# bayespy/bayespy

Hardware: AMD Instinct MI355X
Metric: VB iterations/sec, PCA N=10000000 D=128 K=32 (higher is better)
Workload: dtype f64

## Files before the change

### bayespy_amd/csrc/vmp_common.h

```cpp
#pragma once

#include <hip/hip_runtime.h>
#include <stdint.h>
#include <stdio.h>
#include <string.h>
#include <math.h>

#include "../../include/vmp_hip.h"

#define VMP_EV_RING 64

constexpr int VMP_NME = 16;

struct vmp_xpass_desc {
    const double *Y;
    int64_t ldy, N;
    int D, K;
    double *X;
    int64_t ldx;
    int lay;
    const double *A;
    int buf;
};

struct vmp_ctx {
    int device;
    hipStream_t stream;
    int num_cu;
    int timing;
    hipEvent_t ev[3 * VMP_EV_RING];
    int64_t ev_n;
    hipStream_t xs;
    hipEvent_t ev_xfork, ev_xdone;
    int x_pending;
    hipEvent_t ev_xbuf[2];
    int x_buf_pending[2];
    int64_t x_count;
    int xs_cus;
    int x_hold, x_held;
    vmp_xpass_desc x_desc;
    int64_t x_launched, x_superseded;
    double *sweep_ctl;
    int64_t sweeps_enqueued;
    unsigned int *sweep_tickets;
    int64_t sweep_mid_launches;
    unsigned long long *sweep_stamps;
    int sweep_stamp_rows;
    hipStream_t ms[3];
    hipEvent_t me[VMP_NME];
    int gram_pending;
    int gram_D, gram_K;
    double *gram_state;
    double *gram_P;
    void *comm;
    int comm_rank, comm_world;
    void *queue;
    char err[512];
};

enum { VMP_SWEEP_NSTAMP = VMP_PCA_SWEEP_NSTAMP };

enum { VMP_SWEEP_STOP = 0, VMP_SWEEP_L = 1, VMP_SWEEP_EXECUTED = 2, VMP_SWEEP_SKIPPED = 3,
       VMP_SWEEP_CTL_LEN = 8 };

struct vmp_sweep_tail {
    const double *P;
    int nb;
    double *ctl;
    double *slot;
    int first;
    int compare;
    double l0, tol;
    int norder;
    int order[8];
};

int32_t vmp_pca_sweep_covered(int32_t D, int32_t K);
int32_t vmp_pca_launch_sweep_head(vmp_ctx *ctx, int32_t D, int32_t K, int64_t n_total, double x_prec,
                                  double a0t, double b0t, double a0a, double b0a, double *state,
                                  const double *stop);
int32_t vmp_pca_launch_sweep_tail(vmp_ctx *ctx, int32_t D, int32_t K, int64_t n_total, double x_prec,
                                  double a0t, double b0t, double a0a, double b0a, double *state,
                                  const vmp_sweep_tail &t);

int32_t vmp_pca_launch_sweep_mid(vmp_ctx *ctx, int32_t D, int32_t K, int64_t n_total, double x_prec,
                                 double a0t, double b0t, double a0a, double b0a, double *state,
                                 double *P, const vmp_sweep_tail &t, unsigned int *ticket, int32_t wide,
                                 unsigned long long *stamps);
int32_t vmp_pca_launch_sweep_head_wide(vmp_ctx *ctx, int32_t D, int32_t K, int64_t n_total,
                                       double x_prec, double a0t, double b0t, double a0a, double b0a,
                                       double *state);
int32_t vmp_pca_launch_gram_fast(vmp_ctx *ctx, int32_t D, int32_t K, double *state, double *P,
                                 int32_t wide);

int32_t vmp_pca_ensure_gram(vmp_ctx *ctx);
int32_t vmp_pca_launch_held(vmp_ctx *ctx);

int32_t vmp_queue_flush(vmp_ctx *ctx);
int32_t vmp_queue_commit(vmp_ctx *ctx);
int32_t destroy_small_queue(vmp_ctx *ctx);
extern const char *vmp_flush_cause;
#define VMP_FLUSH_SMALL(ctx)                                   \
    do {                                                       \
        if ((ctx) && (ctx)->queue) {                           \
            vmp_flush_cause = __func__;                        \
            const int32_t rc__ = vmp_queue_flush(ctx);         \
            if (rc__ != VMP_OK) return rc__;                   \
        }                                                      \
    } while (0)

static inline hipEvent_t *vmp_next_events(vmp_ctx *ctx)
// ... 258 lines not shown
```

### bayespy_amd/csrc/vmp_ctx.hip

```cpp
#include "vmp_common.h"

#include <new>

static char g_err[512] = "no context";

namespace {
struct tune_entry { char key[32]; int value; };
tune_entry g_tune[128];
int g_ntune = 0;
bool g_tune_env = false;
}

extern "C" char **environ;

static void tune_from_env()
{
    g_tune_env = true;
    for (char **e = environ; e && *e; ++e) {
        if (strncmp(*e, "VMP_TUNE_", 9) != 0) continue;
        const char *eq = strchr(*e, '=');
        if (!eq) continue;
        const size_t len = (size_t)(eq - (*e + 9));
        if (len == 0 || len >= sizeof(g_tune[0].key) || g_ntune >= (int)(sizeof(g_tune) / sizeof(g_tune[0])))
            continue;
// ... 52 lines not shown
    vmp_ctx *ctx = new (std::nothrow) vmp_ctx();
    if (!ctx) return VMP_ERR_HIP;
    ctx->device = device;
    ctx->stream = (hipStream_t)stream;
    ctx->timing = 0;
    ctx->err[0] = 0;
    for (int i = 0; i < 3 * VMP_EV_RING; ++i) ctx->ev[i] = nullptr;
    ctx->ev_n = 0;
    ctx->xs = nullptr;
    ctx->ev_xfork = ctx->ev_xdone = nullptr;
    ctx->x_pending = 0;
    ctx->x_buf_pending[0] = ctx->x_buf_pending[1] = 0;
    ctx->x_count = 0;
    ctx->ev_xbuf[0] = ctx->ev_xbuf[1] = nullptr;
    ctx->xs_cus = 0;
    ctx->x_hold = ctx->x_held = 0;
    ctx->x_launched = ctx->x_superseded = 0;
    ctx->sweep_ctl = nullptr;
    ctx->sweeps_enqueued = 0;
    ctx->sweep_tickets = nullptr;
    ctx->sweep_mid_launches = 0;
    ctx->sweep_stamps = nullptr;
    ctx->sweep_stamp_rows = 0;
    for (int i = 0; i < 3; ++i) ctx->ms[i] = nullptr;
    for (int i = 0; i < VMP_NME; ++i) ctx->me[i] = nullptr;
    ctx->comm = nullptr;
    ctx->queue = nullptr;
    ctx->comm_rank = 0;
    ctx->comm_world = 1;
    VMP_HIP_CHECK(ctx, hipSetDevice(device));
    int cu = 0;
    VMP_HIP_CHECK(ctx, hipDeviceGetAttribute(&cu, hipDeviceAttributeMultiprocessorCount, device));
    ctx->num_cu = cu > 0 ? cu : 256;
    *out = ctx;
    return VMP_OK;
}

int32_t vmp_ctx_destroy(vmp_ctx *ctx)
{
    if (!ctx) return VMP_OK;
    (void)destroy_small_queue(ctx);
    (void)vmp_comm_destroy(ctx);
    (void)vmp_pca_launch_held(ctx);
    for (int i = 0; i < 3 * VMP_EV_RING; ++i)
        if (ctx->ev[i]) (void)hipEventDestroy(ctx->ev[i]);
    if (ctx->xs) {
        (void)hipStreamSynchronize(ctx->xs);
        (void)hipStreamDestroy(ctx->xs);
    }
    for (int i = 0; i < 3; ++i)
        if (ctx->ms[i]) {
            (void)hipStreamSynchronize(ctx->ms[i]);
            (void)hipStreamDestroy(ctx->ms[i]);
        }
    for (int i = 0; i < VMP_NME; ++i)
        if (ctx->me[i]) (void)hipEventDestroy(ctx->me[i]);
    if (ctx->sweep_ctl) (void)hipFree(ctx->sweep_ctl);
    if (ctx->sweep_tickets) (void)hipFree(ctx->sweep_tickets);
    if (ctx->sweep_stamps) (void)hipFree(ctx->sweep_stamps);
    if (ctx->ev_xfork) (void)hipEventDestroy(ctx->ev_xfork);
    if (ctx->ev_xdone) (void)hipEventDestroy(ctx->ev_xdone);
    for (int i = 0; i < 2; ++i)
        if (ctx->ev_xbuf[i]) (void)hipEventDestroy(ctx->ev_xbuf[i]);
    delete ctx;
    return VMP_OK;
}

int32_t vmp_ctx_set_stream(vmp_ctx *ctx, void *stream)
{
    if (!ctx) return VMP_ERR_INVALID;
    if ((hipStream_t)stream != ctx->stream) VMP_FLUSH_SMALL(ctx);
    ctx->stream = (hipStream_t)stream;
    return VMP_OK;
}

int32_t vmp_ctx_sync(vmp_ctx *ctx)
{
    if (!ctx) return VMP_ERR_INVALID;
    VMP_FLUSH_SMALL(ctx);
    {
        const int32_t rcg = vmp_pca_ensure_gram(ctx);
        if (rcg != VMP_OK) return rcg;
// ... 261 lines not shown
```

### bayespy_amd/csrc/vmp_pca.hip

```cpp
#include "vmp_common.h"
#include "vmp_stop_rule.h"

namespace {

constexpr int TN = 32;
constexpr int SZ = TN + 2;
constexpr int NT = 256;
constexpr int MAX_KP = 64;
constexpr int MAX_DP = 256;

inline int pow2_blocks(int x, int unit)
{
    int b = (x + unit - 1) / unit;
    int p = 1;
    while (p < b) p <<= 1;
    return p;
}

inline void fill_layout(int D, int K, vmp_pca_layout *L)
{
    const int64_t DP = 32 * pow2_blocks(D, 32);
    const int64_t KP = 16 * pow2_blocks(K, 16);
    int64_t o = 0;
    L->DP = DP;
// ... 1129 lines not shown
    if (rc != VMP_OK) return rc;
    if (!ctx->sweep_ctl) {
        VMP_HIP_CHECK(ctx, hipMalloc(&ctx->sweep_ctl, VMP_SWEEP_CTL_LEN * sizeof(double)));
        VMP_HIP_CHECK(ctx, hipMemsetAsync(ctx->sweep_ctl, 0, VMP_SWEEP_CTL_LEN * sizeof(double),
                                          ctx->stream));
    }
    vmp_pca_layout L;
    fill_layout(D, K, &L);
    double *P = reinterpret_cast<double *>(workspace);
    vmp_sweep_tail t;
    t.P = P;
    t.nb = (int)(L.DP / GR);
    t.ctl = ctx->sweep_ctl;
    t.compare = compare ? 1 : 0;
    t.l0 = l0;
    t.tol = tol;
    t.norder = norder;
    for (int i = 0; i < 8; ++i) t.order[i] = i < norder ? order[i] : -1;
    const bool ticket = n > 1 && ((uintptr_t)state % 16) == 0 &&
                        vmp_tune_get("pca_sweep_ticket", env_int("VMP_PCA_SWEEP_TICKET", 1, 0, 1));
    int wide = vmp_tune_get("pca_sweep_wide", env_int("VMP_PCA_SWEEP_WIDE", 1, 0, 1)) ? 1 : 0;
    if (wide && vmp_tune_get("pca_sweep_local_pxx", env_int("VMP_PCA_SWEEP_LOCAL_PXX", 1, 0, 1)))
        wide = 2;
    const bool stamps = ticket && vmp_tune_get("pca_sweep_stamps", 0);
    if (stamps) {
        const size_t bytes = (size_t)VMP_PCA_MAX_SWEEPS * VMP_SWEEP_NSTAMP * sizeof(unsigned long long);
        if (!ctx->sweep_stamps) VMP_HIP_CHECK(ctx, hipMalloc(&ctx->sweep_stamps, bytes));
        VMP_HIP_CHECK(ctx, hipMemsetAsync(ctx->sweep_stamps, 0,
                                          (size_t)(n - 1) * VMP_SWEEP_NSTAMP * sizeof(unsigned long long),
                                          ctx->stream));
        ctx->sweep_stamp_rows = n - 1;
    }
    if (ticket) {
        if (!ctx->sweep_tickets) {
            VMP_HIP_CHECK(ctx, hipMalloc(&ctx->sweep_tickets,
                                         VMP_PCA_MAX_SWEEPS * sizeof(unsigned int)));
            VMP_HIP_CHECK(ctx, hipMemsetAsync(ctx->sweep_tickets, 0,
                                              VMP_PCA_MAX_SWEEPS * sizeof(unsigned int), ctx->stream));
        }
    }
    bool head_wide = ticket && wide;
    if (head_wide && ctx->x_pending) {
        head_wide = hipEventQuery(ctx->ev_xdone) == hipSuccess;
        (void)hipGetLastError();
    }
    for (int i = 0; i < n; ++i) {
        const double *stop = i == 0 ? nullptr : ctx->sweep_ctl;
        const bool last = i + 1 == n;
        if (i == 0 && head_wide) {
            rc = vmp_pca_launch_sweep_head_wide(ctx, D, K, n_total, x_prec, a0_tau, b0_tau, a0_alpha,
                                                b0_alpha, state);
            if (rc != VMP_OK) return rc;
        } else if (!ticket || i == 0) {
            rc = vmp_pca_launch_sweep_head(ctx, D, K, n_total, x_prec, a0_tau, b0_tau, a0_alpha,
                                           b0_alpha, state, stop);
            if (rc != VMP_OK) return rc;
        }
        if (last) {
            rc = issue_xpass(ctx, Y, ldy, N, D, K, X, ldx, state, workspace, lay);
            if (rc != VMP_OK) return rc;
        } else {
            ctx->x_superseded += 1;
        }
        t.slot = ring + (int64_t)i * VMP_PCA_SWEEP_SLOT;
        t.first = i == 0;
        if (ticket && !last) {
            rc = vmp_pca_launch_sweep_mid(ctx, D, K, n_total, x_prec, a0_tau, b0_tau, a0_alpha,
                                          b0_alpha, state, P, t, ctx->sweep_tickets + i, wide,
                                          stamps ? ctx->sweep_stamps + (size_t)i * VMP_SWEEP_NSTAMP
                                                 : nullptr);
            if (rc != VMP_OK) return rc;
            ctx->sweep_mid_launches += 1;
        } else {
            rc = run_gram_stats(ctx, L, D, K, state, P, ctx->stream, stop, false);
            if (rc != VMP_OK) return rc;
            rc = vmp_pca_launch_sweep_tail(ctx, D, K, n_total, x_prec, a0_tau, b0_tau, a0_alpha,
                                           b0_alpha, state, t);
            if (rc != VMP_OK) return rc;
        }
        ctx->sweeps_enqueued += 1;
    }
    return VMP_OK;
}

int32_t vmp_pca_sweep_counts(vmp_ctx *ctx, int64_t *enqueued, int64_t *executed, int64_t *skipped)
{
    VMP_REQUIRE(ctx, ctx, VMP_ERR_INVALID, "null argument");
    double c[VMP_SWEEP_CTL_LEN] = {0.0};
    if (ctx->sweep_ctl) {
        VMP_HIP_CHECK(ctx, hipStreamSynchronize(ctx->stream));
        VMP_HIP_CHECK(ctx, hipMemcpy(c, ctx->sweep_ctl, sizeof(c), hipMemcpyDeviceToHost));
    }
    if (enqueued) *enqueued = ctx->sweeps_enqueued;
// ... 65 lines not shown
```

### bayespy_amd/csrc/vmp_pca_small.hip

```cpp
#include "vmp_common.h"
#include "vmp_sweep.h"
#include "vmp_stop_rule.h"

#include <stdlib.h>

namespace {


struct small_args {
    vmp_pca_layout L;
    int D, K;
    double n_total, x_prec, a0t, b0t, a0a, b0a;
    int has_mean;
};

__device__ inline double ww_centred(const small_args &a, const double *st, int k)
{
    const vmp_pca_layout &L = a.L;
    double v = st[L.off_Sww + k * L.KP + k];
    if (a.has_mean) v += st[L.off_mstat + L.KP + k] - 2.0 * st[L.off_mstat + k];
    return v;
}

__device__ inline double sxx_total(const double *st, const vmp_pca_layout &L, double n_total,
                                   int i, int j)
{
    const double *S = st + L.off_S;
// ... 81 lines not shown
        vmp_sweep::sweep_upto<0>(T, (n + 3) / 4, l15, l4, prod, ld, isbad);
#pragma unroll
        for (int tr = 0; tr < KP / 16; ++tr)
#pragma unroll
            for (int tc = 0; tc < KP / 16; ++tc)
#pragma unroll
                for (int r = 0; r < 4; ++r) {
                    const int row = 16 * tr + l4 + 4 * r, col = 16 * tc + l15;
                    M[row * LDM + col] = (row < 4 * ((n + 3) / 4) && col < 4 * ((n + 3) / 4))
                                             ? -T[tr][tc][r] : T[tr][tc][r];
                }
        if (l == 0) {
            *logdet = vmp_sweep::sweep_logdet(prod, ld);
            if (isbad) *bad = 1;
        }
    } else {
        side();
    }
    __syncthreads();
}

enum { SP_ENTRY = 0, SP_LDS_FILLED, SP_SYX, SP_PXX, SP_TICKET, SP_ACQUIRE,
       SP_T_PARTIALS, SP_T_LOADS, SP_T_PXX, SP_T_BLOCKSUMS, SP_T_TAU_ALPHA, SP_T_BOUND, SP_T_RING,
       SP_H_LAMBDA, SP_H_INV1, SP_H_W, SP_H_SWW, SP_H_INV2, SP_H_A, SP_COUNT };
static_assert(SP_COUNT <= VMP_SWEEP_NSTAMP, "stamp row length");
struct stamps_off {
    __device__ __forceinline__ void operator()(int) const {}
    __device__ __forceinline__ void drain() const {}
};
struct stamps_on {
    unsigned long long *t;
    __device__ __forceinline__ void operator()(int i) const
    {
        if (threadIdx.x == 0) t[i] = wall_clock64();
    }
    __device__ __forceinline__ void drain() const { asm volatile("s_waitcnt vmcnt(0)" ::: "memory"); }
};

template <int KP, int NTQ>
struct small_lds {
    static constexpr int LDM = KP + 1;
    static constexpr int RB = (KP == 64) ? 16 : 32;
    double M[KP * LDM];
    double Sb[RB * LDM];
    double Wb[RB * LDM];
    double red[NTQ / 64 + 1];
    double logdet;
    int bad;
};

template <int KP, int NTQ>
__device__ void op_update_w(const small_args &a, double *st, small_lds<KP, NTQ> &s)
{
    constexpr int LDM = KP + 1, RB = small_lds<KP, NTQ>::RB, E = KP * KP / NTQ;
    const vmp_pca_layout &L = a.L;
    const int tid = threadIdx.x, D = a.D, K = a.K;
    const double tau = st[L.off_tau + 2];
// ... 514 lines not shown

template <int KP>
__global__ void __launch_bounds__(NTF, 5)
pca_head_fast_kernel(small_args a, double *st, const double *stop)
{
    if (stop && stop[VMP_SWEEP_STOP] != 0.0) return;
    pca_head_body<KP, false>(a, st, nullptr, nullptr, nullptr, 0.0);
}

constexpr int GB = 32;
constexpr int GRA = 8;
constexpr int TAIL_PLAIN = 0, TAIL_GRAM = 1, TAIL_SWEEP = 2;
template <int KP>
struct alignas(16) tail_lds {
    double Sw[KP * (KP + 1)];
    double Cx[KP * (KP + 1)];
    double Sx[KP * (KP + 1)];
    double al[4 * KP];
    double sc[8];
    double red[NTF / 64 + 1];
    double stop;
};
static_assert(sizeof(tail_lds<16>) % 16 == 0 && sizeof(tail_lds<32>) % 16 == 0, "tail_lds size");
template <int KP, int MODE, bool WIDE = false, class STAMP = stamps_off, bool LOCAL = false>
__device__ __forceinline__ void pca_tail_body(const small_args &a, double *st, const vmp_sweep_tail *sw,
                                              tail_lds<KP> &s, double *SW = nullptr,
                                              const STAMP &stamp = STAMP(), const double *AL = nullptr)
{
    static_assert(!WIDE || MODE == TAIL_SWEEP, "the wide tail is a sweep tail");
    static_assert(!LOCAL || WIDE, "sum <x><x>^T is formed locally by the wide tail only");
    constexpr bool GRAM = (MODE == TAIL_GRAM);
    constexpr int LDM = KP + 1, E = KP * KP / NTF;
    extern __shared__ __align__(16) double gl[];
    double *Sw = s.Sw, *Cx = s.Cx, *Sx = s.Sx, *al = s.al, *sc = s.sc, *red = s.red;
    const lay32 L(a.L);
    const int tid = threadIdx.x, D = a.D, K = a.K;
    if constexpr (MODE == TAIL_SWEEP && !LOCAL) {
        if (!sw->first && sw->ctl[VMP_SWEEP_STOP] != 0.0) {
            if (tid == 0) {
                sw->slot[7] = 0.0;
                sw->ctl[VMP_SWEEP_SKIPPED] += 1.0;
            }
            return;
        }
    }
    __builtin_amdgcn_s_setprio(3);
    double t1 = 0.0;
    double sxx[E];
#pragma unroll
    for (int m = 0; m < E; ++m) sxx[m] = 0.0;
    constexpr int NW = WIDE ? FAST_D * KP / NTF : 1;
    double ww[NW], wy[NW], es0[WIDE ? E : 1], es1[WIDE ? E : 1];
    if constexpr (WIDE) {
// ... 228 lines not shown
        }
#pragma unroll
        for (int i = 0; i < B; ++i)
#pragma unroll
            for (int j = 0; j < B; ++j) {
                const int k = ki + 16 * i, k2 = ji + 16 * j;
                const bool in = (k < K && k2 < K);
                const double x = in ? (acc[0][i][j] + acc[1][i][j]) + (acc[2][i][j] + acc[3][i][j]) : 0.0;
                st[L.off_S + (L.DP + k) * KP + k2] = x;
                Sx[k * LDM + k2] = x;
            }
        __syncthreads();
        stamp(SP_T_PXX);
    }
    double t2 = 0.0, trx = 0.0;
#pragma unroll
    for (int m = 0; m < E; ++m) {
        const int e = tid + m * NTF;
        const int i = e / KP, j = e % KP;
        const double sxx = a.n_total * Cx[i * LDM + j] + 0.5 * (Sx[i * LDM + j] + Sx[j * LDM + i]);
        t2 += Sw[i * LDM + j] * sxx;
        if (i == j) trx += sxx;
    }
    t1 = block_sum<NTF>(t1, red);
    t2 = block_sum<NTF>(t2, red);
    trx = block_sum<NTF>(trx, red);
    stamp(SP_T_BLOCKSUMS);
    const double resid = sc[4] - 2.0 * t1 + t2;
    if (tid == 64) {
        const double ta = a.a0t + 0.5 * (double)D * a.n_total;
        const double tb = a.b0t + 0.5 * resid;
        sc[0] = ta;
        sc[1] = tb;
        sc[2] = ta / tb;
        sc[3] = sf_digamma(ta) - sf_log(tb);
        st[L.off_tau + 0] = ta;
        st[L.off_tau + 1] = tb;
        st[L.off_tau + 2] = sc[2];
        st[L.off_tau + 3] = sc[3];
        st[L.off_scal + 2] = resid;
        if (!(tb > 0.0)) st[L.off_scal + 3] = (double)VMP_ERR_FLOATING;
        if constexpr (MODE == TAIL_SWEEP)
            sc[7] = !(tb > 0.0) ? (double)VMP_ERR_FLOATING : st[L.off_scal + 3];
        red[NTF / 64] = gamma_elbo(a.a0t, a.b0t, ta, tb, sc[2], sc[3]);
    }
    double sla = 0.0, saw = 0.0, lal = 0.0;
    if (tid < K) {
        const double aa = a.a0a + 0.5 * (double)D;
        const double ab = a.b0a + 0.5 * Sw[tid * LDM + tid];
        const double am = aa / ab, alg = sf_digamma(aa) - sf_log(ab);
        al[0 * KP + tid] = aa;
// ... 222 lines not shown
        for (int m = 0; m < E; ++m) {
            const int e = tid + m * NTF;
            const int k = e / KP, k2 = e % KP;
            double s = 0.0;
            if (k < K && k2 < K) {
#pragma unroll
                for (int r = 0; r < GRA; ++r)
                    s = __builtin_fma(As[k * LA + r0 + r], Ss[r * LDS_S + k2], s);
            }
            Pb[e] = s;
        }
    }
}

template <int KP>
__global__ void __launch_bounds__(NTF)
pca_gram_wide_kernel(vmp_pca_layout L, int D, int K, double *st, double *P)
{
    extern __shared__ __align__(16) double gl[];
    gram_phase_a_wide<KP>(L, D, K, st, P, gl, blockIdx.x);
}

template <int KP, class STAMP>
__device__ __forceinline__ void pca_head_wide(const small_args &a, double *st, double *M, double *T,
                                              const double *alm, double tau, double *SW,
                                              const STAMP &stamp)
{
    constexpr int LDM = KP + 1, E = KP * KP / NTF, KT = KP / 16;
    constexpr int WT = FAST_D / 16 * KT / 4;
    constexpr int ST = (KT * KT + 3) / 4;
    __shared__ double logdet;
    __shared__ int bad;
    const lay32 L(a.L);
    const int tid = threadIdx.x, D = a.D, K = a.K, DP = (int)L.DP;
    const int nr = (D + 31) / 32 * 32;
    const int nt = nr / 16 * KT;
    const int w = tid >> 6, l15 = tid & 15, l4 = (tid & 63) >> 4;
    if (tid == 0) bad = 0;
    {
        double lam[E];
#pragma unroll
        for (int m = 0; m < E; ++m) {
            const int e = tid + m * NTF;
            const int i = e / KP, j = e % KP;
            double x = (i == j) ? 1.0 : 0.0;
            if (i < K && j < K) {
                x = tau * (a.n_total * M[i * LDM + j] + 0.5 * (T[i * LDM + j] + T[j * LDM + i]));
                if (i == j) x += alm[i];
            }
            lam[m] = x;
        }
        __syncthreads();
#pragma unroll
        for (int m = 0; m < E; ++m) {
            const int e = tid + m * NTF;
            M[(e / KP) * LDM + (e % KP)] = lam[m];
        }
    }
    stamp(SP_H_LAMBDA);
    sweep_inverse<KP>(M, K, &logdet, &bad);
    stamp(SP_H_INV1);
#pragma unroll
    for (int m = 0; m < E; ++m) {
        const int e = tid + m * NTF;
        const int i = e / KP, j = e % KP;
        if (i < K && j < K) st[L.off_CW + i * KP + j] = M[i * LDM + j];
    }
    if (tid == 0) st[L.off_scal + 0] = logdet;
    v4f64 wt[WT];
#pragma unroll
    for (int t = 0; t < WT; ++t) {
        const int tile = w + 4 * t;
        if (tile < nt)
            wt[t] = wave_tile_mma(SW + (tile / KT) * 16 * LDM, LDM, 1, M + (tile % KT) * 16, LDM, 1, KP);
    }
    __syncthreads();
#pragma unroll
    for (int t = 0; t < WT; ++t) {
        const int tile = w + 4 * t;
        if (tile < nt) {
#pragma unroll
            for (int r = 0; r < 4; ++r) {
                const int row = (tile / KT) * 16 + l4 + 4 * r, k = (tile % KT) * 16 + l15;
// ... 52 lines not shown
        if (tile < nt) {
            const int tk = tile % KT, td = tile / KT;
            const v4f64 acc = wave_tile_mma(M + tk * 16 * LDM, LDM, 1, SW + td * 16 * LDM, 1, LDM, KP);
#pragma unroll
            for (int r = 0; r < 4; ++r) {
                const int k = tk * 16 + l4 + 4 * r, d = td * 16 + l15;
                if (k < K && d < D) st[L.off_A + k * DP + d] = tau * acc[r];
            }
        }
    }
    if (tid == 0) {
        st[L.off_scal + 1] = logdet;
        if (bad) st[L.off_scal + 3] = (double)VMP_ERR_NOT_POSDEF;
    }
    stamp.drain();
    stamp(SP_H_A);
}

__host__ __device__ inline size_t sweep_local_lds(int KP, int DP)
{
    return ((size_t)KP * (DP + 2) + (size_t)DP * (KP + 1) + 2) * sizeof(double);
}

template <int KP, bool WIDE, bool LOCAL, class STAMP>
__device__ __forceinline__ void pca_sweep_mid_body(const small_args &a, double *st, double *P,
                                                   const vmp_sweep_tail &sw, unsigned int *ticket,
                                                   const STAMP &stamp)
{
    static_assert(!LOCAL || WIDE, "sum <x><x>^T is formed locally beside the wide bodies only");
    extern __shared__ __align__(16) double gl[];
    __shared__ tail_lds<KP> ts;
    const int tid = threadIdx.x;
    if (!sw.first && sw.ctl[VMP_SWEEP_STOP] != 0.0) {
        if (blockIdx.x == 0 && tid == 0) {
            sw.slot[7] = 0.0;
            sw.ctl[VMP_SWEEP_SKIPPED] += 1.0;
        }
        return;
    }
    stamp(SP_ENTRY);
    if constexpr (WIDE)
        gram_phase_a_wide<KP, STAMP, !LOCAL>(a.L, a.D, a.K, st, P, gl, blockIdx.x, stamp);
    else
        gram_phase_a<KP>(a.L, a.D, a.K, st, P, gl, blockIdx.x, stamp);
    asm volatile("s_waitcnt vmcnt(0)" ::: "memory");
    __syncthreads();
    stamp(SP_PXX);
    const int na = LOCAL ? KP * ((int)a.L.DP + 2) : 0;
    double *SW = gl + na;
    unsigned int *word = reinterpret_cast<unsigned int *>(LOCAL ? SW + (int)a.L.DP * (KP + 1) : gl);
    if (tid == 0) {
        __builtin_amdgcn_fence(__ATOMIC_RELEASE, "agent");
        asm volatile("s_waitcnt vmcnt(0)" ::: "memory");
        *word = __hip_atomic_fetch_add(ticket, 1u, __ATOMIC_RELAXED, __HIP_MEMORY_SCOPE_AGENT);
    }
    __syncthreads();
    if (*word != gridDim.x - 1) return;
    stamp(SP_TICKET);
    if (tid == 0) {
        __builtin_amdgcn_fence(__ATOMIC_ACQUIRE, "agent");
        asm volatile("s_waitcnt vmcnt(0)" ::: "memory");
        *ticket = 0u;
    }
    __syncthreads();
    stamp(SP_ACQUIRE);
    pca_tail_body<KP, TAIL_SWEEP, WIDE, STAMP, LOCAL>(a, st, &sw, ts, SW, stamp, gl);
    __syncthreads();
    if (ts.stop != 0.0) return;
    if constexpr (WIDE)
        pca_head_wide<KP>(a, st, ts.Cx, ts.Sx, ts.al + 2 * KP, ts.sc[2], SW, stamp);
    else
        pca_head_body<KP, true>(a, st, ts.Cx, ts.Sx, ts.al + 2 * KP, ts.sc[2], stamp);
}

template <int KP, bool WIDE, bool LOCAL>
__global__ void __launch_bounds__(NTF)
pca_sweep_mid_kernel(small_args a, double *st, double *P, vmp_sweep_tail sw, unsigned int *ticket)
{
    pca_sweep_mid_body<KP, WIDE, LOCAL>(a, st, P, sw, ticket, stamps_off());
}

template <int KP, bool WIDE, bool LOCAL>
__global__ void __launch_bounds__(NTF)
pca_sweep_mid_stamped_kernel(small_args a, double *st, double *P, vmp_sweep_tail sw,
                             unsigned int *ticket, unsigned long long *out)
{
    __shared__ unsigned long long stl[VMP_SWEEP_NSTAMP];
    if (threadIdx.x < VMP_SWEEP_NSTAMP) stl[threadIdx.x] = 0;
    __syncthreads();
    const stamps_on stamp{stl};
    pca_sweep_mid_body<KP, WIDE, LOCAL>(a, st, P, sw, ticket, stamp);
    if (threadIdx.x == 0 && stl[SP_T_LOADS] != 0)
        for (int i = 0; i < VMP_SWEEP_NSTAMP; ++i) out[i] = stl[i];
}

template <int KP>
__global__ void __launch_bounds__(NTF)
pca_head_wide_kernel(small_args a, double *st)
{
    constexpr int LDM = KP + 1, E = KP * KP / NTF, NW = FAST_D * KP / NTF;
    __shared__ __align__(16) double M[KP * LDM], T[KP * LDM], SW[FAST_D * LDM], alm[KP];
    const lay32 L(a.L);
    const int tid = threadIdx.x, D = a.D, K = a.K;
    const int n = D * KP, nsw = (D + 31) / 32 * 32 * KP;
    double cx[E], sx[E], wy[NW];
#pragma unroll
    for (int m = 0; m < E; ++m) {
        const int e = tid + m * NTF;
        const int i = e / KP, j = e % KP;
        const bool in = (i < K && j < K);
        cx[m] = in ? st[L.off_CX + i * KP + j] : 0.0;
        sx[m] = in ? st[L.off_S + (L.DP + i) * KP + j] : 0.0;
    }
#pragma unroll
    for (int j = 0; j < NW; ++j) {
        const int e = tid + j * NTF;
        wy[j] = (e < n && e % KP < K) ? st[L.off_S + e] : 0.0;
    }
    const double tau = st[L.off_tau + 2];
    if (tid < KP) alm[tid] = tid < K ? st[L.off_alpha + 2 * KP + tid] : 0.0;
#pragma unroll
    for (int m = 0; m < E; ++m) {
        const int e = tid + m * NTF;
        M[(e / KP) * LDM + (e % KP)] = cx[m];
        T[(e / KP) * LDM + (e % KP)] = sx[m];
    }
#pragma unroll
    for (int j = 0; j < NW; ++j) {
        const int e = tid + j * NTF;
        if (e < nsw) SW[(e / KP) * LDM + (e % KP)] = wy[j];
    }
    __syncthreads();
    pca_head_wide<KP>(a, st, M, T, alm, tau, SW, stamps_off());
}

bool fast_small_enabled()
{
    static const int v = getenv("VMP_PCA_FAST_SMALL") ? atoi(getenv("VMP_PCA_FAST_SMALL")) : 1;
    return v != 0;
}

int32_t fill_small_args(vmp_ctx *ctx, small_args &a, int32_t D, int32_t K, int64_t n_total,
                        double x_prec, double a0t, double b0t, double a0a, double b0a)
{
    const int32_t rc = vmp_pca_get_layout(D, K, &a.L);
    VMP_REQUIRE(ctx, rc == VMP_OK, rc, "unsupported dims D=%d K=%d", D, K);
    a.D = D;
    a.K = K;
    a.n_total = (double)n_total;
    a.x_prec = x_prec;
    a.a0t = a0t; a.b0t = b0t; a.a0a = a0a; a.b0a = b0a;
    a.has_mean = 0;
    return VMP_OK;
}

template <int O0, int O1, int O2>
// ... 185 lines not shown
    const int nb = (int)(L.DP / GRA);
    if (wide) {
        const size_t ldw = gram_phase_a_wide_lds((int)L.KP, (int)L.DP);
        if (L.KP == 16)
            hipLaunchKernelGGL(pca_gram_wide_kernel<16>, dim3(nb), dim3(NTF), ldw, ctx->stream, L, D, K,
                               state, P);
        else
            hipLaunchKernelGGL(pca_gram_wide_kernel<32>, dim3(nb), dim3(NTF), ldw, ctx->stream, L, D, K,
                               state, P);
        VMP_HIP_CHECK(ctx, hipGetLastError());
        return VMP_OK;
    }
    const size_t lds = gram_phase_a_lds((int)L.KP, (int)L.DP);
    if (L.KP == 16)
        hipLaunchKernelGGL(pca_gram_fast_kernel<16>, dim3(nb), dim3(NTF), lds, ctx->stream, L, D, K,
                           state, P);
    else
        hipLaunchKernelGGL(pca_gram_fast_kernel<32>, dim3(nb), dim3(NTF), lds, ctx->stream, L, D, K,
                           state, P);
    VMP_HIP_CHECK(ctx, hipGetLastError());
    return VMP_OK;
}

template <int KP, bool WIDE, bool LOCAL>
static int32_t launch_mid(vmp_ctx *ctx, const small_args &a, double *state, double *P,
                          const vmp_sweep_tail &t, unsigned int *ticket, unsigned long long *stamps)
{
    static bool raised[2][64] = {{false}};
    const int dev = ctx->device & 63, s = stamps ? 1 : 0;
    if (!raised[s][dev]) {
        const void *f = stamps ? (const void *)pca_sweep_mid_stamped_kernel<KP, WIDE, LOCAL>
                               : (const void *)pca_sweep_mid_kernel<KP, WIDE, LOCAL>;
        VMP_HIP_CHECK(ctx, hipFuncSetAttribute(f, hipFuncAttributeMaxDynamicSharedMemorySize,
                                               96 * 1024));
        raised[s][dev] = true;
    }
    const size_t lds = LOCAL ? sweep_local_lds((int)a.L.KP, (int)a.L.DP)
                       : WIDE ? gram_phase_a_wide_lds((int)a.L.KP, (int)a.L.DP)
                              : gram_phase_a_lds((int)a.L.KP, (int)a.L.DP);
    const dim3 nb((unsigned)(a.L.DP / GRA));
    if (stamps)
        hipLaunchKernelGGL((pca_sweep_mid_stamped_kernel<KP, WIDE, LOCAL>), nb, dim3(NTF), lds, ctx->stream, a,
                           state, P, t, ticket, stamps);
    else
        hipLaunchKernelGGL((pca_sweep_mid_kernel<KP, WIDE, LOCAL>), nb, dim3(NTF), lds, ctx->stream, a, state,
                           P, t, ticket);
    VMP_HIP_CHECK(ctx, hipGetLastError());
    return VMP_OK;
}

int32_t vmp_pca_launch_sweep_mid(vmp_ctx *ctx, int32_t D, int32_t K, int64_t n_total, double x_prec,
                                 double a0t, double b0t, double a0a, double b0a, double *state,
                                 double *P, const vmp_sweep_tail &t, unsigned int *ticket, int32_t wide,
                                 unsigned long long *stamps)
{
    small_args a;
    const int32_t rc = fill_small_args(ctx, a, D, K, n_total, x_prec, a0t, b0t, a0a, b0a);
    if (rc != VMP_OK) return rc;
    if (a.L.KP == 16)
        return wide == 2 ? launch_mid<16, true, true>(ctx, a, state, P, t, ticket, stamps)
               : wide    ? launch_mid<16, true, false>(ctx, a, state, P, t, ticket, stamps)
                         : launch_mid<16, false, false>(ctx, a, state, P, t, ticket, stamps);
    return wide == 2 ? launch_mid<32, true, true>(ctx, a, state, P, t, ticket, stamps)
           : wide    ? launch_mid<32, true, false>(ctx, a, state, P, t, ticket, stamps)
                     : launch_mid<32, false, false>(ctx, a, state, P, t, ticket, stamps);
}

int32_t vmp_pca_launch_sweep_head_wide(vmp_ctx *ctx, int32_t D, int32_t K, int64_t n_total,
                                       double x_prec, double a0t, double b0t, double a0a, double b0a,
                                       double *state)
{
    small_args a;
    const int32_t rc = fill_small_args(ctx, a, D, K, n_total, x_prec, a0t, b0t, a0a, b0a);
    if (rc != VMP_OK) return rc;
    if (a.L.KP == 16)
        hipLaunchKernelGGL(pca_head_wide_kernel<16>, dim3(1), dim3(NTF), 0, ctx->stream, a, state);
    else
        hipLaunchKernelGGL(pca_head_wide_kernel<32>, dim3(1), dim3(NTF), 0, ctx->stream, a, state);
    VMP_HIP_CHECK(ctx, hipGetLastError());
    return VMP_OK;
}

extern "C" {

int32_t vmp_pca_small_ops(vmp_ctx *ctx, int32_t D, int32_t K, int64_t n_total, double x_prec,
                          double a0_tau, double b0_tau, double a0_alpha, double b0_alpha,
                          int32_t nops, const int32_t *ops, double *state)
{
// ... 49 lines not shown
```

Baseline: 23200.

## Defer sweep bound evaluation into a side wave overlapping the head inverse

In the fused sweep-mid kernel, the tail now skips the serial bound and stop-rule computation and hands it to a second wavefront. That wave computes the bound and stop rule while sweep_inverse runs, using hyperparameter-only constants (digamma, lgamma, logs) precomputed once by a small kernel and cached by key. Block reductions for the three tail sums are also cut to one barrier with wave sums. The aim is to take transcendental math and the bound off the critical path of each sweep. The cost is that the head starts speculatively and must check the stop flag after the inverse, which adds more template variants and complexity.

```diff
diff --git a/bayespy_amd/csrc/vmp_common.h b/bayespy_amd/csrc/vmp_common.h
--- a/bayespy_amd/csrc/vmp_common.h
+++ b/bayespy_amd/csrc/vmp_common.h
@@ -46,6 +46,9 @@
     int64_t sweep_mid_launches;
     unsigned long long *sweep_stamps;
     int sweep_stamp_rows;
+    double *sweep_sf;
+    double sweep_sf_key[7];
+    int sweep_sf_valid;
     hipStream_t ms[3];
     hipEvent_t me[VMP_NME];
     int gram_pending;
@@ -63,6 +66,9 @@
 enum { VMP_SWEEP_STOP = 0, VMP_SWEEP_L = 1, VMP_SWEEP_EXECUTED = 2, VMP_SWEEP_SKIPPED = 3,
        VMP_SWEEP_CTL_LEN = 8 };
 
+enum { VMP_SWEEP_SF_TAU = 0, VMP_SWEEP_SF_ALPHA = 4, VMP_SWEEP_SF_LOG2PI = 8, VMP_SWEEP_SF_LOGXPREC = 9,
+       VMP_SWEEP_SF_LEN = 10 };
+
 struct vmp_sweep_tail {
     const double *P;
     int nb;
@@ -86,7 +92,9 @@
 int32_t vmp_pca_launch_sweep_mid(vmp_ctx *ctx, int32_t D, int32_t K, int64_t n_total, double x_prec,
                                  double a0t, double b0t, double a0a, double b0a, double *state,
                                  double *P, const vmp_sweep_tail &t, unsigned int *ticket, int32_t wide,
-                                 unsigned long long *stamps);
+                                 unsigned long long *stamps, int32_t stamp_level);
+int32_t vmp_pca_sweep_constants(vmp_ctx *ctx, int32_t D, int32_t K, int64_t n_total, double x_prec,
+                                double a0t, double b0t, double a0a, double b0a);
 int32_t vmp_pca_launch_sweep_head_wide(vmp_ctx *ctx, int32_t D, int32_t K, int64_t n_total,
                                        double x_prec, double a0t, double b0t, double a0a, double b0a,
                                        double *state);
diff --git a/bayespy_amd/csrc/vmp_ctx.hip b/bayespy_amd/csrc/vmp_ctx.hip
--- a/bayespy_amd/csrc/vmp_ctx.hip
+++ b/bayespy_amd/csrc/vmp_ctx.hip
@@ -98,6 +98,8 @@
     ctx->sweep_mid_launches = 0;
     ctx->sweep_stamps = nullptr;
     ctx->sweep_stamp_rows = 0;
+    ctx->sweep_sf = nullptr;
+    ctx->sweep_sf_valid = 0;
     for (int i = 0; i < 3; ++i) ctx->ms[i] = nullptr;
     for (int i = 0; i < VMP_NME; ++i) ctx->me[i] = nullptr;
     ctx->comm = nullptr;
@@ -134,6 +136,7 @@
     if (ctx->sweep_ctl) (void)hipFree(ctx->sweep_ctl);
     if (ctx->sweep_tickets) (void)hipFree(ctx->sweep_tickets);
     if (ctx->sweep_stamps) (void)hipFree(ctx->sweep_stamps);
+    if (ctx->sweep_sf) (void)hipFree(ctx->sweep_sf);
     if (ctx->ev_xfork) (void)hipEventDestroy(ctx->ev_xfork);
     if (ctx->ev_xdone) (void)hipEventDestroy(ctx->ev_xdone);
     for (int i = 0; i < 2; ++i)
diff --git a/bayespy_amd/csrc/vmp_pca.hip b/bayespy_amd/csrc/vmp_pca.hip
--- a/bayespy_amd/csrc/vmp_pca.hip
+++ b/bayespy_amd/csrc/vmp_pca.hip
@@ -1175,7 +1175,14 @@
     int wide = vmp_tune_get("pca_sweep_wide", env_int("VMP_PCA_SWEEP_WIDE", 1, 0, 1)) ? 1 : 0;
     if (wide && vmp_tune_get("pca_sweep_local_pxx", env_int("VMP_PCA_SWEEP_LOCAL_PXX", 1, 0, 1)))
         wide = 2;
-    const bool stamps = ticket && vmp_tune_get("pca_sweep_stamps", 0);
+    if (wide == 2 && vmp_tune_get("pca_sweep_defer", env_int("VMP_PCA_SWEEP_DEFER", 1, 0, 1)))
+        wide = 3;
+    if (ticket && wide == 3) {
+        rc = vmp_pca_sweep_constants(ctx, D, K, n_total, x_prec, a0_tau, b0_tau, a0_alpha, b0_alpha);
+        if (rc != VMP_OK) return rc;
+    }
+    const int stamp_level = ticket ? vmp_tune_get("pca_sweep_stamps", 0) : 0;
+    const bool stamps = stamp_level != 0;
     if (stamps) {
         const size_t bytes = (size_t)VMP_PCA_MAX_SWEEPS * VMP_SWEEP_NSTAMP * sizeof(unsigned long long);
         if (!ctx->sweep_stamps) VMP_HIP_CHECK(ctx, hipMalloc(&ctx->sweep_stamps, bytes));
@@ -1221,7 +1228,7 @@
             rc = vmp_pca_launch_sweep_mid(ctx, D, K, n_total, x_prec, a0_tau, b0_tau, a0_alpha,
                                           b0_alpha, state, P, t, ctx->sweep_tickets + i, wide,
                                           stamps ? ctx->sweep_stamps + (size_t)i * VMP_SWEEP_NSTAMP
-                                                 : nullptr);
+                                                 : nullptr, stamp_level);
             if (rc != VMP_OK) return rc;
             ctx->sweep_mid_launches += 1;
         } else {
diff --git a/bayespy_amd/csrc/vmp_pca_small.hip b/bayespy_amd/csrc/vmp_pca_small.hip
--- a/bayespy_amd/csrc/vmp_pca_small.hip
+++ b/bayespy_amd/csrc/vmp_pca_small.hip
@@ -3,6 +3,8 @@
 #include "vmp_stop_rule.h"
 
 #include <stdlib.h>
+#include <string.h>
+#include <type_traits>
 
 namespace {
 
@@ -130,17 +132,24 @@
 
 enum { SP_ENTRY = 0, SP_LDS_FILLED, SP_SYX, SP_PXX, SP_TICKET, SP_ACQUIRE,
        SP_T_PARTIALS, SP_T_LOADS, SP_T_PXX, SP_T_BLOCKSUMS, SP_T_TAU_ALPHA, SP_T_BOUND, SP_T_RING,
-       SP_H_LAMBDA, SP_H_INV1, SP_H_W, SP_H_SWW, SP_H_INV2, SP_H_A, SP_COUNT };
-static_assert(SP_COUNT <= VMP_SWEEP_NSTAMP, "stamp row length");
+       SP_H_LAMBDA, SP_H_INV1, SP_H_W, SP_H_SWW, SP_H_INV2, SP_H_A, SP_COUNT,
+       SP_S_STATE = SP_COUNT, SP_S_RING, SP_COUNT2 };
+static_assert(SP_COUNT2 <= VMP_SWEEP_NSTAMP, "stamp row length");
 struct stamps_off {
     __device__ __forceinline__ void operator()(int) const {}
+    __device__ __forceinline__ void side(int) const {}
     __device__ __forceinline__ void drain() const {}
 };
 struct stamps_on {
     unsigned long long *t;
+    int level;
     __device__ __forceinline__ void operator()(int i) const
     {
         if (threadIdx.x == 0) t[i] = wall_clock64();
+    }
+    __device__ __forceinline__ void side(int i) const
+    {
+        if (level >= 2 && threadIdx.x == 64) t[i] = wall_clock64();
     }
     __device__ __forceinline__ void drain() const { asm volatile("s_waitcnt vmcnt(0)" ::: "memory"); }
 };
@@ -701,13 +710,15 @@
     double stop;
 };
 static_assert(sizeof(tail_lds<16>) % 16 == 0 && sizeof(tail_lds<32>) % 16 == 0, "tail_lds size");
-template <int KP, int MODE, bool WIDE = false, class STAMP = stamps_off, bool LOCAL = false>
+template <int KP, int MODE, bool WIDE = false, class STAMP = stamps_off, bool LOCAL = false,
+          bool DEFER = false>
 __device__ __forceinline__ void pca_tail_body(const small_args &a, double *st, const vmp_sweep_tail *sw,
                                               tail_lds<KP> &s, double *SW = nullptr,
                                               const STAMP &stamp = STAMP(), const double *AL = nullptr)
 {
     static_assert(!WIDE || MODE == TAIL_SWEEP, "the wide tail is a sweep tail");
     static_assert(!LOCAL || WIDE, "sum <x><x>^T is formed locally by the wide tail only");
+    static_assert(!DEFER || LOCAL, "the bound is deferred behind the local wide tail only");
     constexpr bool GRAM = (MODE == TAIL_GRAM);
     constexpr int LDM = KP + 1, E = KP * KP / NTF;
     extern __shared__ __align__(16) double gl[];
@@ -982,11 +993,63 @@
         t2 += Sw[i * LDM + j] * sxx;
         if (i == j) trx += sxx;
     }
-    t1 = block_sum<NTF>(t1, red);
-    t2 = block_sum<NTF>(t2, red);
-    trx = block_sum<NTF>(trx, red);
+    if constexpr (DEFER) {
+        double *r3 = al + 3 * KP;
+        static_assert(KP >= 3 * (NTF / 64), "twelve words");
+        t1 = wave_sum(t1);
+        t2 = wave_sum(t2);
+        trx = wave_sum(trx);
+        if ((tid & 63) == 0) {
+            r3[tid >> 6] = t1;
+            r3[NTF / 64 + (tid >> 6)] = t2;
+            r3[2 * (NTF / 64) + (tid >> 6)] = trx;
+        }
+        __syncthreads();
+        t1 = t2 = trx = 0.0;
+#pragma unroll
+        for (int i = 0; i < NTF / 64; ++i) {
+            t1 += r3[i];
+            t2 += r3[NTF / 64 + i];
+            trx += r3[2 * (NTF / 64) + i];
+        }
+    } else {
+        t1 = block_sum<NTF>(t1, red);
+        t2 = block_sum<NTF>(t2, red);
+        trx = block_sum<NTF>(trx, red);
+    }
     stamp(SP_T_BLOCKSUMS);
     const double resid = sc[4] - 2.0 * t1 + t2;
+    if constexpr (DEFER) {
+        if (tid == 64) {
+            const double ta = a.a0t + 0.5 * (double)D * a.n_total;
+            const double tb = a.b0t + 0.5 * resid;
+            sc[0] = ta;
+            sc[1] = tb;
+            sc[2] = ta / tb;
+            red[0] = resid;
+            red[1] = trx;
+            st[L.off_tau + 0] = ta;
+            st[L.off_tau + 1] = tb;
+            st[L.off_tau + 2] = sc[2];
+            st[L.off_scal + 2] = resid;
+            if (!(tb > 0.0)) st[L.off_scal + 3] = (double)VMP_ERR_FLOATING;
+        }
+        if (tid < K) {
+            const double aa = a.a0a + 0.5 * (double)D;
+            const double ab = a.b0a + 0.5 * Sw[tid * LDM + tid];
+            const double am = aa / ab;
+            al[0 * KP + tid] = aa;
+            al[1 * KP + tid] = ab;
+            al[2 * KP + tid] = am;
+            st[L.off_alpha + 0 * KP + tid] = aa;
+            st[L.off_alpha + 1 * KP + tid] = ab;
+            st[L.off_alpha + 2 * KP + tid] = am;
+        }
+        stamp(SP_T_TAU_ALPHA);
+        stamp(SP_T_BOUND);
+        stamp(SP_T_RING);
+        return;
+    }
     if (tid == 64) {
         const double ta = a.a0t + 0.5 * (double)D * a.n_total;
         const double tb = a.b0t + 0.5 * resid;
@@ -1255,10 +1318,89 @@
 }
 
 template <int KP, class STAMP>
+struct defer_side {
+    const small_args &a;
+    double *st;
+    const vmp_sweep_tail &sw;
+    tail_lds<KP> &s;
+    const double *sf;
+    const STAMP &stamp;
+    __device__ __forceinline__ void operator()() const
+    {
+        constexpr int LDM = KP + 1;
+        if (threadIdx.x >= 128) return;
+        const lay32 L(a.L);
+        const int l = threadIdx.x - 64, D = a.D, K = a.K;
+        const bool isa = l < K;
+        const int k = isa ? l : 0;
+        const double a0 = isa ? a.a0a : a.a0t, b0 = isa ? a.b0a : a.b0t;
+        const double av = isa ? s.al[0 * KP + k] : s.sc[0];
+        const double bv = isa ? s.al[1 * KP + k] : s.sc[1];
+        const double mean = isa ? s.al[2 * KP + k] : s.sc[2];
+        const double *c = sf + (isa ? VMP_SWEEP_SF_ALPHA : VMP_SWEEP_SF_TAU);
+        const double dg = c[0], lga = c[1], lga0 = c[2], logb0 = c[3];
+        const double logb = sf_log(bv);
+        const double logx = dg - logb;
+        const double g_p = a0 * logb0 - lga0;
+        const double g_q = av * logb - lga;
+        const double g = g_p - g_q + (bv - b0) * mean + (a0 - av) * logx;
+        if (isa) st[L.off_alpha + 3 * KP + k] = logx;
+        if (l == 32) st[L.off_tau + 3] = logx;
+        stamp.side(SP_S_STATE);
+        const double sla = 0.0 + wave_sum(isa ? logx : 0.0);
+        const double saw = 0.0 + wave_sum(isa ? mean * s.Sw[k * LDM + k] : 0.0);
+        const double lal = 0.0 + wave_sum(isa ? g : 0.0);
+        const double logtau = __shfl(logx, 32, 64), Lt = __shfl(g, 32, 64);
+        if (l == 0) {
+            const double tau = s.sc[2], resid = s.red[0], trx = s.red[1];
+            const double Dd = (double)D, Kd = (double)K;
+            const double LY = Dd * a.n_total * (-0.5 * sf[VMP_SWEEP_SF_LOG2PI] + 0.5 * logtau)
+                              - 0.5 * tau * resid;
+            const double LX = -0.5 * a.x_prec * trx
+                              + a.n_total * (0.5 * Kd * sf[VMP_SWEEP_SF_LOGXPREC] - 0.5 * s.sc[6] + 0.5 * Kd);
+            const double LW = 0.5 * Dd * sla - 0.5 * saw + Dd * (-0.5 * s.sc[5] + 0.5 * Kd);
+            st[L.off_L + 0] = LY;
+            st[L.off_L + 1] = LX;
+            st[L.off_L + 2] = LW;
+            st[L.off_L + 3] = Lt;
+            st[L.off_L + 4] = lal;
+            st[L.off_L + 5] = LY + LX + LW + Lt + lal;
+            const double status = !(s.sc[1] > 0.0) ? (double)VMP_ERR_FLOATING : st[L.off_scal + 3];
+            double *slot = sw.slot;
+            slot[0] = LY;
+            slot[1] = LX;
+            slot[2] = LW;
+            slot[3] = Lt;
+            slot[4] = lal;
+            slot[5] = LY + LX + LW + Lt + lal;
+            slot[6] = status;
+            slot[7] = 1.0;
+            double *al = s.al;
+            al[0] = LY;
+            al[1] = LX;
+            al[2] = LW;
+            al[3] = Lt;
+            al[4] = lal;
+            const double Lb = vmp_bound_sum(al, sw.order, sw.norder);
+            const double L0 = sw.first ? sw.l0 : sw.ctl[VMP_SWEEP_L];
+            int stop = status != 0.0;
+            if (sw.compare && vmp_stop_rule(Lb, L0, sw.tol)) stop = 1;
+            sw.ctl[VMP_SWEEP_STOP] = stop ? 1.0 : 0.0;
+            s.stop = stop ? 1.0 : 0.0;
+            sw.ctl[VMP_SWEEP_L] = Lb;
+            sw.ctl[VMP_SWEEP_EXECUTED] += 1.0;
+        }
+        stamp.side(SP_S_RING);
+    }
+};
+
+template <int KP, class STAMP, class SIDE = no_side>
 __device__ __forceinline__ void pca_head_wide(const small_args &a, double *st, double *M, double *T,
                                               const double *alm, double tau, double *SW,
-                                              const STAMP &stamp)
-{
+                                              const STAMP &stamp, const SIDE &side = SIDE(),
+                                              const double *stopw = nullptr)
+{
+    constexpr bool DEFER = !std::is_same<SIDE, no_side>::value;
     constexpr int LDM = KP + 1, E = KP * KP / NTF, KT = KP / 16;
     constexpr int WT = FAST_D / 16 * KT / 4;
     constexpr int ST = (KT * KT + 3) / 4;
@@ -1291,7 +1433,12 @@
         }
     }
     stamp(SP_H_LAMBDA);
-    sweep_inverse<KP>(M, K, &logdet, &bad);
+    if constexpr (DEFER) {
+        sweep_inverse<KP>(M, K, &logdet, &bad, side);
+        if (*stopw != 0.0) return;
+    } else {
+        sweep_inverse<KP>(M, K, &logdet, &bad);
+    }
     stamp(SP_H_INV1);
 #pragma unroll
     for (int m = 0; m < E; ++m) {
@@ -1390,12 +1537,13 @@
     return ((size_t)KP * (DP + 2) + (size_t)DP * (KP + 1) + 2) * sizeof(double);
 }
 
-template <int KP, bool WIDE, bool LOCAL, class STAMP>
+template <int KP, bool WIDE, bool LOCAL, bool DEFER, class STAMP>
 __device__ __forceinline__ void pca_sweep_mid_body(const small_args &a, double *st, double *P,
                                                    const vmp_sweep_tail &sw, unsigned int *ticket,
-                                                   const STAMP &stamp)
+                                                   const double *sf, const STAMP &stamp)
 {
     static_assert(!LOCAL || WIDE, "sum <x><x>^T is formed locally beside the wide bodies only");
+    static_assert(!DEFER || LOCAL, "the bound is deferred behind the local wide tail only");
     extern __shared__ __align__(16) double gl[];
     __shared__ tail_lds<KP> ts;
     const int tid = threadIdx.x;
@@ -1432,8 +1580,13 @@
     }
     __syncthreads();
     stamp(SP_ACQUIRE);
-    pca_tail_body<KP, TAIL_SWEEP, WIDE, STAMP, LOCAL>(a, st, &sw, ts, SW, stamp, gl);
+    pca_tail_body<KP, TAIL_SWEEP, WIDE, STAMP, LOCAL, DEFER>(a, st, &sw, ts, SW, stamp, gl);
     __syncthreads();
+    if constexpr (DEFER) {
+        const defer_side<KP, STAMP> side{a, st, sw, ts, sf, stamp};
+        pca_head_wide<KP>(a, st, ts.Cx, ts.Sx, ts.al + 2 * KP, ts.sc[2], SW, stamp, side, &ts.stop);
+        return;
+    }
     if (ts.stop != 0.0) return;
     if constexpr (WIDE)
         pca_head_wide<KP>(a, st, ts.Cx, ts.Sx, ts.al + 2 * KP, ts.sc[2], SW, stamp);
@@ -1441,23 +1594,24 @@
         pca_head_body<KP, true>(a, st, ts.Cx, ts.Sx, ts.al + 2 * KP, ts.sc[2], stamp);
 }
 
-template <int KP, bool WIDE, bool LOCAL>
+template <int KP, bool WIDE, bool LOCAL, bool DEFER = false>
 __global__ void __launch_bounds__(NTF)
-pca_sweep_mid_kernel(small_args a, double *st, double *P, vmp_sweep_tail sw, unsigned int *ticket)
-{
-    pca_sweep_mid_body<KP, WIDE, LOCAL>(a, st, P, sw, ticket, stamps_off());
-}
-
-template <int KP, bool WIDE, bool LOCAL>
+pca_sweep_mid_kernel(small_args a, double *st, double *P, vmp_sweep_tail sw, unsigned int *ticket,
+                     const double *sf)
+{
+    pca_sweep_mid_body<KP, WIDE, LOCAL, DEFER>(a, st, P, sw, ticket, sf, stamps_off());
+}
+
+template <int KP, bool WIDE, bool LOCAL, bool DEFER = false>
 __global__ void __launch_bounds__(NTF)
 pca_sweep_mid_stamped_kernel(small_args a, double *st, double *P, vmp_sweep_tail sw,
-                             unsigned int *ticket, unsigned long long *out)
+                             unsigned int *ticket, const double *sf, unsigned long long *out, int level)
 {
     __shared__ unsigned long long stl[VMP_SWEEP_NSTAMP];
     if (threadIdx.x < VMP_SWEEP_NSTAMP) stl[threadIdx.x] = 0;
     __syncthreads();
-    const stamps_on stamp{stl};
-    pca_sweep_mid_body<KP, WIDE, LOCAL>(a, st, P, sw, ticket, stamp);
+    const stamps_on stamp{stl, level};
+    pca_sweep_mid_body<KP, WIDE, LOCAL, DEFER>(a, st, P, sw, ticket, sf, stamp);
     if (threadIdx.x == 0 && stl[SP_T_LOADS] != 0)
         for (int i = 0; i < VMP_SWEEP_NSTAMP; ++i) out[i] = stl[i];
 }
@@ -1500,6 +1654,29 @@
     }
     __syncthreads();
     pca_head_wide<KP>(a, st, M, T, alm, tau, SW, stamps_off());
+}
+
+__global__ void __launch_bounds__(64)
+pca_sweep_sf_kernel(small_args a, double *sf)
+{
+    const int l = threadIdx.x;
+    if (l >= VMP_SWEEP_SF_LEN) return;
+    const double ta = a.a0t + 0.5 * (double)a.D * a.n_total;
+    const double aa = a.a0a + 0.5 * (double)a.D;
+    double v;
+    switch (l) {
+    case VMP_SWEEP_SF_TAU + 0: v = sf_digamma(ta); break;
+    case VMP_SWEEP_SF_TAU + 1: v = sf_lgamma(ta); break;
+    case VMP_SWEEP_SF_TAU + 2: v = sf_lgamma(a.a0t); break;
+    case VMP_SWEEP_SF_TAU + 3: v = sf_log(a.b0t); break;
+    case VMP_SWEEP_SF_ALPHA + 0: v = sf_digamma(aa); break;
+    case VMP_SWEEP_SF_ALPHA + 1: v = sf_lgamma(aa); break;
+    case VMP_SWEEP_SF_ALPHA + 2: v = sf_lgamma(a.a0a); break;
+    case VMP_SWEEP_SF_ALPHA + 3: v = sf_log(a.b0a); break;
+    case VMP_SWEEP_SF_LOG2PI: v = sf_log(2.0 * M_PI); break;
+    default: v = sf_log(a.x_prec); break;
+    }
+    sf[l] = v;
 }
 
 bool fast_small_enabled()
@@ -1731,15 +1908,18 @@
     return VMP_OK;
 }
 
-template <int KP, bool WIDE, bool LOCAL>
+template <int KP, bool WIDE, bool LOCAL, bool DEFER = false>
 static int32_t launch_mid(vmp_ctx *ctx, const small_args &a, double *state, double *P,
-                          const vmp_sweep_tail &t, unsigned int *ticket, unsigned long long *stamps)
-{
+                          const vmp_sweep_tail &t, unsigned int *ticket, unsigned long long *stamps,
+                          int stamp_level)
+{
+    VMP_REQUIRE(ctx, !DEFER || ctx->sweep_sf, VMP_ERR_INVALID,
+                "the deferred sweep needs vmp_pca_sweep_constants first");
     static bool raised[2][64] = {{false}};
     const int dev = ctx->device & 63, s = stamps ? 1 : 0;
     if (!raised[s][dev]) {
-        const void *f = stamps ? (const void *)pca_sweep_mid_stamped_kernel<KP, WIDE, LOCAL>
-                               : (const void *)pca_sweep_mid_kernel<KP, WIDE, LOCAL>;
+        const void *f = stamps ? (const void *)pca_sweep_mid_stamped_kernel<KP, WIDE, LOCAL, DEFER>
+                               : (const void *)pca_sweep_mid_kernel<KP, WIDE, LOCAL, DEFER>;
         VMP_HIP_CHECK(ctx, hipFuncSetAttribute(f, hipFuncAttributeMaxDynamicSharedMemorySize,
                                                96 * 1024));
         raised[s][dev] = true;
@@ -1749,11 +1929,12 @@
                               : gram_phase_a_lds((int)a.L.KP, (int)a.L.DP);
     const dim3 nb((unsigned)(a.L.DP / GRA));
     if (stamps)
-        hipLaunchKernelGGL((pca_sweep_mid_stamped_kernel<KP, WIDE, LOCAL>), nb, dim3(NTF), lds, ctx->stream, a,
-                           state, P, t, ticket, stamps);
+        hipLaunchKernelGGL((pca_sweep_mid_stamped_kernel<KP, WIDE, LOCAL, DEFER>), nb, dim3(NTF), lds,
+                           ctx->stream, a, state, P, t, ticket, (const double *)ctx->sweep_sf, stamps,
+                           stamp_level);
     else
-        hipLaunchKernelGGL((pca_sweep_mid_kernel<KP, WIDE, LOCAL>), nb, dim3(NTF), lds, ctx->stream, a, state,
-                           P, t, ticket);
+        hipLaunchKernelGGL((pca_sweep_mid_kernel<KP, WIDE, LOCAL, DEFER>), nb, dim3(NTF), lds, ctx->stream, a,
+                           state, P, t, ticket, (const double *)ctx->sweep_sf);
     VMP_HIP_CHECK(ctx, hipGetLastError());
     return VMP_OK;
 }
@@ -1761,18 +1942,39 @@
 int32_t vmp_pca_launch_sweep_mid(vmp_ctx *ctx, int32_t D, int32_t K, int64_t n_total, double x_prec,
                                  double a0t, double b0t, double a0a, double b0a, double *state,
                                  double *P, const vmp_sweep_tail &t, unsigned int *ticket, int32_t wide,
-                                 unsigned long long *stamps)
+                                 unsigned long long *stamps, int32_t stamp_level)
 {
     small_args a;
     const int32_t rc = fill_small_args(ctx, a, D, K, n_total, x_prec, a0t, b0t, a0a, b0a);
     if (rc != VMP_OK) return rc;
+    const int sl = stamp_level;
     if (a.L.KP == 16)
-        return wide == 2 ? launch_mid<16, true, true>(ctx, a, state, P, t, ticket, stamps)
-               : wide    ? launch_mid<16, true, false>(ctx, a, state, P, t, ticket, stamps)
-                         : launch_mid<16, false, false>(ctx, a, state, P, t, ticket, stamps);
-    return wide == 2 ? launch_mid<32, true, true>(ctx, a, state, P, t, ticket, stamps)
-           : wide    ? launch_mid<32, true, false>(ctx, a, state, P, t, ticket, stamps)
-                     : launch_mid<32, false, false>(ctx, a, state, P, t, ticket, stamps);
+        return wide == 3 ? launch_mid<16, true, true, true>(ctx, a, state, P, t, ticket, stamps, sl)
+               : wide == 2 ? launch_mid<16, true, true>(ctx, a, state, P, t, ticket, stamps, sl)
+               : wide      ? launch_mid<16, true, false>(ctx, a, state, P, t, ticket, stamps, sl)
+                           : launch_mid<16, false, false>(ctx, a, state, P, t, ticket, stamps, sl);
+    return wide == 3 ? launch_mid<32, true, true, true>(ctx, a, state, P, t, ticket, stamps, sl)
+           : wide == 2 ? launch_mid<32, true, true>(ctx, a, state, P, t, ticket, stamps, sl)
+           : wide      ? launch_mid<32, true, false>(ctx, a, state, P, t, ticket, stamps, sl)
+                       : launch_mid<32, false, false>(ctx, a, state, P, t, ticket, stamps, sl);
+}
+
+int32_t vmp_pca_sweep_constants(vmp_ctx *ctx, int32_t D, int32_t K, int64_t n_total, double x_prec,
+                                double a0t, double b0t, double a0a, double b0a)
+{
+    small_args a;
+    const int32_t rc = fill_small_args(ctx, a, D, K, n_total, x_prec, a0t, b0t, a0a, b0a);
+    if (rc != VMP_OK) return rc;
+    const double key[7] = {a0t, b0t, a0a, b0a, (double)D, (double)n_total, x_prec};
+    if (ctx->sweep_sf && ctx->sweep_sf_valid && memcmp(key, ctx->sweep_sf_key, sizeof(key)) == 0)
+        return VMP_OK;
+    if (!ctx->sweep_sf) VMP_HIP_CHECK(ctx, hipMalloc(&ctx->sweep_sf, VMP_SWEEP_SF_LEN * sizeof(double)));
+    ctx->sweep_sf_valid = 0;
+    hipLaunchKernelGGL(pca_sweep_sf_kernel, dim3(1), dim3(64), 0, ctx->stream, a, ctx->sweep_sf);
+    VMP_HIP_CHECK(ctx, hipGetLastError());
+    memcpy(ctx->sweep_sf_key, key, sizeof(key));
+    ctx->sweep_sf_valid = 1;
+    return VMP_OK;
 }
 
 int32_t vmp_pca_launch_sweep_head_wide(vmp_ctx *ctx, int32_t D, int32_t K, int64_t n_total,
```

Result: faster. 26260, median of 6 (+13.2%).
